# Darkkey/erlamsa

Measured on AMD Instinct MI355X. Metric: mutated_MB_per_s, higher is better.
Workload: dtype u8 (byte edits) + f64 (AS183 draws)

## Files before the change

### erlamsa_amd/csrc/eh_fuse.h

```cpp
#pragma once
#include "eh_field.h"

namespace eh {

struct FNode { uint32_t fo, fc, to, tc; };

EH_DEV uint32_t wave_sort64(uint32_t key) {
  const uint32_t l = (uint32_t)EH_LANE;
#pragma unroll
  for (uint32_t k2 = 2; k2 <= 64; k2 <<= 1) {
#pragma unroll
    for (uint32_t j = k2 >> 1; j > 0; j >>= 1) {
      uint32_t other = (uint32_t)__shfl_xor((int)key, (int)j);
      bool up = (l & k2) == 0 || k2 == 64, lower = (l & j) == 0;
      bool take_min = lower == up;
      uint32_t mn = key < other ? key : other, mx = key < other ? other : key;
      key = take_min ? mn : mx;
    }
  }
  return key;
}
EH_DEV uint32_t lanes_le(uint32_t v, uint32_t cnt, uint32_t x) {
  uint32_t lo = 0;
#pragma unroll
  for (uint32_t s = 32; s > 0; s >>= 1) { uint32_t t = (uint32_t)__shfl((int)v, (int)((lo + s - 1) & 63)); if (lo + s <= cnt && t <= x) lo += s; }
  { uint32_t t = (uint32_t)__shfl((int)v, (int)(lo & 63)); if (lo < cnt && t <= x) lo++; }
  return lo;
}
EH_DEV uint32_t lanes_lt(uint32_t v, uint32_t cnt, uint32_t x) { uint32_t r = lanes_le(v, cnt, x ? x - 1 : 0u); return x == 0 ? 0u : r; }

EH_DEV uint64_t wave_sum64(uint64_t v) {
#pragma unroll
  for (int d = 32; d > 0; d >>= 1) v += ((uint64_t)(uint32_t)__shfl_xor((int)(uint32_t)(v >> 32), d) << 32) | (uint32_t)__shfl_xor((int)(uint32_t)v, d);
  return uni64(v);
}
}
#include "eh_fuse_lds.h"
namespace eh {
#define FUSE_UNROLL 4
struct FuseGen { EH_G FNode* nd; wptr F; wptr T; };

EH_DEV uint32_t fuse_round(cbptr A, uint32_t la, cbptr B, uint32_t lb, const FuseGen& g, uint32_t nn, const FuseGen& o, uint32_t par, bool sym, uint64_t* entries) {
  const int l = EH_LANE;
  const bool asc = par == 0;
  uint64_t le = 0;
  uint32_t cn = 0, cf = 0, ct = 0;
  uint32_t k0 = 0;
  while (k0 < nn) {
    uint32_t k = k0 + (uint32_t)l;
    FNode nd = {0, 0, 0, 0};
    if (k < nn) nd = g.nd[k];
    if (sym) { nd.to = nd.fo; nd.tc = nd.fc; }
    bool valid = k < nn;
    bool big = valid && (nd.fc > 64 || nd.tc > 64);
    bool one = valid && nd.fc == 1 && nd.tc == 1;
    unsigned long long vm = __ballot(valid), bm = __ballot(big), om = __ballot(one);
    uint32_t nvalid = (uint32_t)__popcll(vm);
    uint32_t nones = ~om == 0ull ? 64u : (uint32_t)__builtin_ctzll(~om);
    if (nones > nvalid) nones = nvalid;
    if (nones >= 16 || (nones > 0 && nones == nvalid)) {
      bool in = (uint32_t)l < nones;
      uint32_t p = in ? nd.fo : la, q = in ? nd.to : lb;
      bool special = in && p == la - 1;
      bool same;
      if (sym) same = in && p < la;
      else { uint32_t ba = (in && p < la) ? A[p] : 256u, bb = (in && q < lb) ? B[q] : 257u; same = ba == bb; }
      bool child = special || same;
      bool tkeep = child && !special && q != lb - 1;
      unsigned long long cm = __ballot(child);
      uint32_t ci = (uint32_t)__popcll(cm & ((1ull << l) - 1));
      if (child) {
        FNode c2; c2.fo = special ? la : p + 1; c2.fc = 1; c2.to = special ? lb : q + 1; c2.tc = (special || tkeep) ? 1u : 0u;
        o.nd[cn + ci] = c2;
        le += 1u + c2.tc;
      }
      cn += (uint32_t)__popcll(cm);
      k0 += nones;
      continue;
    }
    if (bm & 1ull) {
      FNode b0; b0.fo = uni(nd.fo); b0.fc = uni(nd.fc); b0.to = uni(nd.to); b0.tc = uni(nd.tc);
      uint32_t* hf = g_fuse_lds; uint32_t* ht = sym ? g_fuse_lds : g_fuse_lds + 256;
      uint32_t* hc = g_fuse_lds + 512; uint32_t* hk = g_fuse_lds + 768;
      for (uint32_t i = l; i < 512; i += 64) g_fuse_lds[i] = 0;
      lanes_sync();
      uint32_t fdb = 0xFFFFFFFFu, fdbefore = 0, tdb = 0xFFFFFFFFu, tdbefore = 0;
      for (int side = 0; side < (sym ? 1 : 2); side++) {
        cbptr S = side ? B : A; uint32_t slen = side ? lb : la;
        uint32_t cnt = side ? b0.tc : b0.fc;
        cwptr P = side ? g.T + b0.to : g.F + b0.fo;
        uint32_t single = side ? b0.to : b0.fo;
        uint32_t* h = side ? ht : hf;
        for (uint32_t base = 0; base < cnt; base += 64 * FUSE_UNROLL) {
          uint32_t pp[FUSE_UNROLL], bt[FUSE_UNROLL]; bool v[FUSE_UNROLL];
#pragma unroll
          for (int u = 0; u < FUSE_UNROLL; u++) {
            uint32_t i = base + 64u * (uint32_t)u + (uint32_t)l; bool in = i < cnt;
            pp[u] = in ? (cnt == 1 ? single : P[i]) : slen; v[u] = in && pp[u] < slen;
          }
#pragma unroll
          for (int u = 0; u < FUSE_UNROLL; u++) { bt[u] = v[u] ? (uint32_t)S[pp[u]] : 0u; if (!asc) bt[u] = 255u - bt[u]; }
#pragma unroll
          for (int u = 0; u < FUSE_UNROLL; u++) {
            unsigned long long lastm = __ballot(v[u] && pp[u] == slen - 1);
            if (lastm) {
              int j = (int)__builtin_ctzll(lastm);
              uint32_t bj = (uint32_t)__builtin_amdgcn_readlane((int)bt[u], j);
              lanes_sync();
              uint32_t before = h[bj] + (uint32_t)__popcll(__ballot(v[u] && bt[u] == bj) & ((1ull << j) - 1));
              if (side) { tdb = bj; tdbefore = before; } else { fdb = bj; fdbefore = before; }
              lanes_sync();
            }
            if (v[u]) atomicAdd(&h[bt[u]], 1u);
          }
        }
      }
      if (sym) { tdb = fdb; tdbefore = fdbefore; }
      lanes_sync();
      uint32_t rf[4], rt[4], ef[4], et[4]; bool ch[4], sp[4];
      uint32_t lc = 0, lf = 0, lt2 = 0;
      bool anyfd = false, anytd = false;
#pragma unroll
      for (int j = 0; j < 4; j++) {
        uint32_t bt = 4u * (uint32_t)l + (uint32_t)j;
        rf[j] = hf[bt]; rt[j] = ht[bt];
        bool fdrop = bt == fdb && (asc ? fdbefore == 0 : fdbefore + 1 == rf[j]);
        bool tdrop = bt == tdb && (asc ? tdbefore == 0 : tdbefore + 1 == rt[j]);
        anyfd |= fdrop; anytd |= tdrop;
        ef[j] = rf[j] - (fdrop ? 1u : 0u); et[j] = rt[j] - (tdrop ? 1u : 0u);
        sp[j] = rf[j] > 0 && ef[j] == 0;
        ch[j] = rf[j] > 0 && (sp[j] || rt[j] > 0);
        if (sp[j]) { ef[j] = 1; et[j] = 1; }
        if (!ch[j]) { ef[j] = 0; et[j] = 0; }
        le += ef[j] + et[j];
        lc += ch[j] ? 1u : 0u; lf += ef[j] > 1 ? ef[j] : 0u; lt2 += et[j] > 1 ? et[j] : 0u;
      }
      const bool fdropped = __ballot(anyfd) != 0, tdropped = __ballot(anytd) != 0;
      uint32_t ic = wave_incl_scan(lc), iff = wave_incl_scan(lf), it = wave_incl_scan(lt2);
      uint32_t oc = cn + ic - lc, of = cf + iff - lf, ot = sym ? of : ct + it - lt2;
      lanes_sync();
#pragma unroll
      for (int j = 0; j < 4; j++) {
        uint32_t bt = 4u * (uint32_t)l + (uint32_t)j;
        bool scat = ch[j] && !sp[j];
        hf[bt] = scat ? of : 0xFFFFFFFFu; if (!sym) ht[bt] = scat ? ot : 0xFFFFFFFFu;
        hc[bt] = scat ? oc : 0xFFFFFFFFu; hk[bt] = (ef[j] == 1 ? 1u : 0u) | (et[j] == 1 ? 2u : 0u);
        if (ch[j]) {
          FNode c2; c2.fo = sp[j] ? la : of; c2.fc = ef[j]; c2.to = sp[j] ? lb : ot; c2.tc = et[j];
          o.nd[oc] = c2;
          oc++; if (ef[j] > 1) of += ef[j]; if (sym) ot = of; else if (et[j] > 1) ot += et[j];
        }
      }
      cn += (uint32_t)__builtin_amdgcn_readlane((int)ic, 63); cf += (uint32_t)__builtin_amdgcn_readlane((int)iff, 63); ct += (uint32_t)__builtin_amdgcn_readlane((int)it, 63);
      wave_sync();
      for (int side = 0; side < (sym ? 1 : 2); side++) {
        cbptr S = side ? B : A; uint32_t slen = side ? lb : la;
        uint32_t cnt = side ? b0.tc : b0.fc;
        cwptr P = side ? g.T + b0.to : g.F + b0.fo;
        uint32_t single = side ? b0.to : b0.fo;
        uint32_t* h = side ? ht : hf; wptr O = side ? o.T : o.F;
        const bool dropped = side ? tdropped : fdropped;
        for (uint32_t base = 0; base < cnt; base += 64 * FUSE_UNROLL) {
          uint32_t ppu[FUSE_UNROLL], btu[FUSE_UNROLL]; bool vu[FUSE_UNROLL];
#pragma unroll
          for (int u = 0; u < FUSE_UNROLL; u++) {
            uint32_t i = base + 64u * (uint32_t)u + (uint32_t)l; bool in = i < cnt;
            ppu[u] = in ? (cnt == 1 ? single : P[i]) : slen; vu[u] = in && ppu[u] < slen;
          }
#pragma unroll
          for (int u = 0; u < FUSE_UNROLL; u++) { btu[u] = vu[u] ? (uint32_t)S[ppu[u]] : 0u; if (!asc) btu[u] = 255u - btu[u]; }
#pragma unroll
          for (int u = 0; u < FUSE_UNROLL; u++) {
            const uint32_t pp = ppu[u], bt = btu[u]; const bool v = vu[u];
            if (base + 64u * (uint32_t)u >= cnt) break;
            bool isdrop = dropped && v && pp == slen - 1;
            bool vv = v && !isdrop;
            unsigned long long eq = __ballot(vv);
#pragma unroll
            for (int bit = 0; bit < 8; bit++) { unsigned long long m = __ballot(vv && ((bt >> bit) & 1u)); eq &= ((bt >> bit) & 1u) ? m : ~m; }
            uint32_t rank = (uint32_t)__popcll(eq & ((1ull << l) - 1)), cntg = (uint32_t)__popcll(eq);
            uint32_t off = vv ? h[bt] : 0xFFFFFFFFu, cidx = vv ? hc[bt] : 0xFFFFFFFFu, kf = vv ? hk[bt] : 0u;
            lanes_sync();
            if (vv && cidx != 0xFFFFFFFFu) {
              bool isone = (kf >> side) & 1u;
              if (isone) { if (side) o.nd[cidx].to = pp + 1; else { o.nd[cidx].fo = pp + 1; if (sym) o.nd[cidx].to = pp + 1; } }
              else { O[off + rank] = pp + 1; if (rank == 0) h[bt] = off + cntg; }
            }
            lanes_sync();
          }
        }
      }
      k0 += 1;
      continue;
    }
    uint32_t cumf = wave_incl_scan(valid && !big ? nd.fc : 0u), cumt = wave_incl_scan(valid && !big ? nd.tc : 0u);
    uint32_t firstbig = bm ? (uint32_t)__builtin_ctzll(bm) : 64u;
    unsigned long long fitm = __ballot(valid && (uint32_t)l < firstbig && cumf <= 64 && cumt <= 64);
    uint32_t nfit = ~fitm == 0ull ? 64u : (uint32_t)__builtin_ctzll(~fitm);
    uint32_t totf = (uint32_t)__builtin_amdgcn_readlane((int)cumf, (int)(nfit - 1)), tott = (uint32_t)__builtin_amdgcn_readlane((int)cumt, (int)(nfit - 1));
    uint32_t key[2], pos[2], tot[2] = {totf, tott};
#pragma unroll
    for (int side = 0; side < 2; side++) {
      if (side == 1 && sym) { key[1] = key[0]; pos[1] = pos[0]; break; }
      cbptr S = side ? B : A; uint32_t slen = side ? lb : la;
      uint32_t cum = side ? cumt : cumf, cntn = side ? nd.tc : nd.fc, offn = side ? nd.to : nd.fo;
      bool in = (uint32_t)l < tot[side];
      uint32_t nj = lanes_le(cum, nfit, (uint32_t)l);
      uint32_t ex = (uint32_t)__shfl((int)(cum - cntn), (int)(nj & 63)), ob = (uint32_t)__shfl((int)offn, (int)(nj & 63)), cj = (uint32_t)__shfl((int)cntn, (int)(nj & 63));
      uint32_t pp = slen;
      if (in) pp = cj == 1 ? ob : (side ? g.T : g.F)[ob + ((uint32_t)l - ex)];
      bool v = in && pp < slen;
      uint32_t bt = v ? (uint32_t)S[pp] : 0u; if (!asc) bt = 255u - bt;
      uint32_t kk = in ? (((nj << 9) | (v ? bt : 511u)) << 6) | (uint32_t)l : 0xFFFFFFFFu;
      uint32_t nxt = (uint32_t)__shfl_down((int)kk, 1);
      uint32_t sk = __ballot(l < 63 && kk > nxt) == 0 ? kk : wave_sort64(kk);
      key[side] = sk; pos[side] = (uint32_t)__shfl((int)pp, (int)(sk & 63u));
    }
    uint32_t gk[2], lead[2], len[2], drops[2]; bool alive[2], isdrop[2];
#pragma unroll
    for (int side = 0; side < 2; side++) {
      if (side == 1 && sym) { gk[1] = gk[0]; lead[1] = lead[0]; len[1] = len[0]; drops[1] = drops[0]; alive[1] = alive[0]; isdrop[1] = isdrop[0]; break; }
      uint32_t slen = side ? lb : la;
      gk[side] = key[side] >> 6;
      alive[side] = (uint32_t)l < tot[side] && (gk[side] & 511u) != 511u;
      uint32_t prevk = (uint32_t)__shfl_up((int)gk[side], 1), nextk = (uint32_t)__shfl_down((int)gk[side], 1);
      bool leader = alive[side] && (l == 0 || prevk != gk[side]);
      bool last = alive[side] && (l == 63 || (uint32_t)l + 1 >= tot[side] || nextk != gk[side]);
      unsigned long long lm = __ballot(leader);
      uint32_t ll = alive[side] ? 63u - (uint32_t)__builtin_clzll(lm & ((2ull << l) - 1)) : 0u;
      unsigned long long after = lm & ~((2ull << ll) - 1);
      unsigned long long am = __ballot(alive[side]);
      uint32_t endl = after ? (uint32_t)__builtin_ctzll(after) : 64u;
      unsigned long long dead_after = ~am & ~((2ull << ll) - 1);
      uint32_t endd = dead_after ? (uint32_t)__builtin_ctzll(dead_after) : 64u;
      uint32_t e = endl < endd ? endl : endd;
      lead[side] = ll; len[side] = alive[side] ? e - ll : 0u;
      isdrop[side] = alive[side] && pos[side] == slen - 1 && (asc ? leader : last);
      unsigned long long dm = __ballot(isdrop[side]);
      unsigned long long runm = (e >= 64 ? ~0ull : ((1ull << e) - 1)) & ~((1ull << ll) - 1);
      drops[side] = alive[side] ? (uint32_t)__popcll(dm & runm) : 0u;
    }
    uint32_t tl = sym ? lead[0] : lanes_lt(gk[1], tott, gk[0]);
    uint32_t tk_at = (uint32_t)__shfl((int)gk[1], (int)(tl & 63)), tlen_at = (uint32_t)__shfl((int)len[1], (int)(tl & 63)), tdr_at = (uint32_t)__shfl((int)drops[1], (int)(tl & 63));
    bool tldrop = __shfl((int)(isdrop[1] ? 1 : 0), (int)(tl & 63)) != 0;
    bool texists = alive[0] && tl < tott && tk_at == gk[0];
    bool fleader = alive[0] && lead[0] == (uint32_t)l;
    uint32_t fcnt = len[0] - drops[0];
    bool special = fleader && fcnt == 0;
    bool child = fleader && (special || texists);
    uint32_t nf = child ? (special ? 1u : fcnt) : 0u, nt = child ? (special ? 1u : (tlen_at - tdr_at)) : 0u;
    uint32_t af = nf > 1 ? nf : 0u, at = nt > 1 ? nt : 0u;
    uint32_t ic = wave_incl_scan(child ? 1u : 0u), iff = wave_incl_scan(af), it = wave_incl_scan(at);
    uint32_t oc = cn + ic - (child ? 1u : 0u), of = cf + iff - af, ot = sym ? of : ct + it - at;
    uint32_t fsurv = (uint32_t)__shfl((int)pos[0], (int)(((uint32_t)l + (isdrop[0] ? 1u : 0u)) & 63));
    uint32_t tsurv = (uint32_t)__shfl((int)pos[1], (int)((tl + (tldrop ? 1u : 0u)) & 63));
    if (child) {
      FNode c2;
      c2.fc = nf; c2.tc = nt;
      c2.fo = special ? la : (nf == 1 ? fsurv + 1 : of);
      c2.to = special ? lb : (nt == 1 ? tsurv + 1 : (nt == 0 ? 0u : ot));
      o.nd[oc] = c2;
      le += nf + nt;
    }
    {
      bool lmulti = __shfl((int)(child && !special && nf > 1 ? 1 : 0), (int)lead[0]) != 0;
      uint32_t lof = (uint32_t)__shfl((int)of, (int)lead[0]);
      bool ldrop = __shfl((int)(isdrop[0] ? 1 : 0), (int)lead[0]) != 0;
      if (alive[0] && lmulti && !isdrop[0]) o.F[lof + ((uint32_t)l - lead[0]) - (ldrop ? 1u : 0u)] = pos[0] + 1;
    }
    if (!sym) {
      uint32_t sl = lanes_lt(gk[0], totf, gk[1]);
      uint32_t sk_at = (uint32_t)__shfl((int)gk[0], (int)(sl & 63));
      bool has = alive[1] && sl < totf && sk_at == gk[1];
      bool smulti = __shfl((int)(child && !special && nt > 1 ? 1 : 0), (int)(sl & 63)) != 0;
      uint32_t sot = (uint32_t)__shfl((int)ot, (int)(sl & 63));
      bool ldrop = __shfl((int)(isdrop[1] ? 1 : 0), (int)lead[1]) != 0;
      if (has && smulti && !isdrop[1]) o.T[sot + ((uint32_t)l - lead[1]) - (ldrop ? 1u : 0u)] = pos[1] + 1;
    }
    cn += (uint32_t)__builtin_amdgcn_readlane((int)ic, 63); cf += (uint32_t)__builtin_amdgcn_readlane((int)iff, 63); ct += (uint32_t)__builtin_amdgcn_readlane((int)it, 63);
    k0 += nfit;
  }
  *entries = wave_sum64(le);
  wave_sync();
  return cn;
}

__device__ bool fuse_jump_stream(Ctx& c, cbptr A, uint32_t la, cbptr B, uint32_t lb, bool sym, uint32_t* from, uint32_t* tpos, uint32_t* rounds);
}
#include "eh_fuse_red.h"
namespace eh {

#ifdef EH_FUSE_INLINE
EH_DEV bool fuse_lists(Ctx& c, cbptr A, uint32_t la, cbptr B, uint32_t lb, bptr* out, uint32_t* outlen) {
#else
__device__ __noinline__ bool fuse_lists(Ctx&, cbptr A, uint32_t la, cbptr B, uint32_t lb, bptr* out, uint32_t* outlen) {
  EH_CTX;
#endif
  const int l = EH_LANE;
  if (la == 0) { *out = (bptr)B; *outlen = lb; return true; }
  if (lb == 0) { *out = (bptr)A; *outlen = la; return true; }
  uint64_t mark = c.ws_used;
  const bool sym = A == B && la == lb;
  EH_PT0;
  uint32_t from = la, tpos = lb;
  uint32_t prof_rounds = 0;
  c.fp_on = 0;
  if ((sym ? (uint64_t)la : (uint64_t)la + lb) > FL_NMAX && !c.work_budget && !(c.p->flags & EH_FLAG_FUSE_NO_REDUCE)) {
    const uint32_t rd = fr_peek_rounds(c.rng);
    if (rd < 64) {
      const uint32_t R = rd + 2u;
      uint32_t la2 = la, lb2 = lb;
      cbptr A2 = fr_reduce(c, A, &la2, R);
      if (!A2) return false;
      cbptr B2 = A2;
      if (sym) lb2 = la2; else { B2 = fr_reduce(c, B, &lb2, R); if (!B2) return false; }
      if ((uint64_t)la2 + lb2 <= ((uint64_t)la + lb) / 4u * 3u) {
        EH_PT(c, 97);
        c.fp_on = 1;
        bool ok;
        if ((sym ? (uint64_t)la2 : (uint64_t)la2 + lb2) <= FL_NMAX && !(c.p->flags & EH_FLAG_FUSE_NO_LDS)) ok = fuse_jump_lds(c, A2, la2, B2, lb2, sym, &from, &tpos, &prof_rounds);
        else ok = fuse_jump_stream(c, A2, la2, B2, lb2, sym, &from, &tpos, &prof_rounds);
        c.fp_on = 0;
        if (!ok) return false;
        EH_PT(c, 54);
        const uint32_t g = c.fp_g, par = g & 1u;
        from = la; tpos = lb;
        if (g == 0) { from = rng_rand(c.rng, la); tpos = rng_rand(c.rng, lb); }
        else if (c.fp_special) { (void)rng_rand(c.rng, 1); (void)rng_rand(c.rng, 1); }
        else {
          cbptr key = A2 + c.fp_keypos;
          const uint32_t limA = la > g ? la - g : 0u, limB = lb > g ? lb - g : 0u;
          const uint32_t fc0 = fr_occ(A, la, limA, key, g, FR_NONE, nullptr), fc = fc0 + c.fp_bA;
          uint32_t pos = 0;
          if (fc > 0) { uint32_t j = rng_rand(c.rng, fc); j = par ? fc - 1u - j : j; if (j < fc0) { (void)fr_occ(A, la, limA, key, g, j, &pos); from = uni(pos) + g; } }
          const uint32_t tc0 = sym ? fc0 : fr_occ(B, lb, limB, key, g, FR_NONE, nullptr), tc = tc0 + c.fp_bB;
          if (tc > 0) { uint32_t j = rng_rand(c.rng, tc); j = par ? tc - 1u - j : j; if (j < tc0) { (void)fr_occ(B, lb, limB, key, g, j, &pos); tpos = uni(pos) + g; } }
        }
        EH_PT(c, 55);
        goto jump;
      }
    }
    EH_PT(c, 98);
    c.ws_used = mark;
  }
  if ((sym ? (uint64_t)la : (uint64_t)la + lb) <= FL_NMAX && !(c.p->flags & EH_FLAG_FUSE_NO_LDS)) {
    if (!fuse_jump_lds(c, A, la, B, lb, sym, &from, &tpos, &prof_rounds)) { if (c.status == CASE_BUDGET) c.ws_used = mark; return false; }
  } else if ((uint64_t)la + lb >= c.p->fuse_stream_min) {
    if (!fuse_jump_stream(c, A, la, B, lb, sym, &from, &tpos, &prof_rounds)) { if (c.status == CASE_BUDGET) c.ws_used = mark; return false; }
  } else {
    FuseGen g[2];
    for (int k = 0; k < 2; k++) {
      g[k].nd = (EH_G FNode*)ws_alloc(c, ((uint64_t)la + 4) * sizeof(FNode));
      g[k].F = (wptr)ws_alloc(c, ((uint64_t)la + 4) * 4);
      g[k].T = sym ? g[k].F : (wptr)ws_alloc(c, ((uint64_t)lb + 4) * 4);
      if (!g[k].nd || !g[k].F || !g[k].T) return false;
    }
    if (la > 1) for (uint32_t i = l; i < la; i += 64) g[0].F[i] = i;
    if (lb > 1 && !sym) for (uint32_t i = l; i < lb; i += 64) g[0].T[i] = i;
    if (l == 0) { FNode n0; n0.fo = 0; n0.fc = la; n0.to = 0; n0.tc = lb; g[0].nd[0] = n0; }
    uint32_t nn = 1, par = 0;
    int64_t fuel = 100000;
    uint64_t gen_entries = (uint64_t)la + lb;
    wave_sync();
    while (true) {
      if (fuel < 0) break;
      if (rng_rand(c.rng, 8) == 0) break;
      if (c.work_budget) {
        c.work += 16ull * gen_entries;
        if (c.work > c.work_budget) { c.status = CASE_BUDGET; c.ws_used = mark; return false; }
      }
      uint32_t nchild = fuse_round(A, la, B, lb, g[par], nn, g[par ^ 1], par, sym, &gen_entries);
      if (nchild == 0) break;
      par ^= 1; nn = nchild;
      fuel -= (int64_t)nchild;
      prof_rounds++;
    }
    uint32_t ni = rng_rand(c.rng, nn);
    FNode nd = g[par].nd[par ? nn - 1 - ni : ni];
    uint32_t fo = uni(nd.fo), fc = uni(nd.fc), to = sym ? fo : uni(nd.to), tc = sym ? fc : uni(nd.tc);
    if (fc > 0) { uint32_t j = rng_rand(c.rng, fc); from = fc == 1 ? fo : uni(g[par].F[fo + (par ? fc - 1 - j : j)]); }
    if (tc > 0) { uint32_t j = rng_rand(c.rng, tc); tpos = tc == 1 ? to : uni(g[par].T[to + (par ? tc - 1 - j : j)]); }
  }
jump:
#ifdef EH_PROF
  {
    uint32_t tot = la + lb, b = 0; while ((256u << b) < tot && b < 13) b++;
    EH_PT(c, 112 + b);
    if (EH_LANE == 0) { atomicAdd(&c.p->prof[2 * 126], (unsigned long long)prof_rounds); atomicAdd(&c.p->prof[2 * 126 + 1], 1ull); }
  }
#endif
  c.ws_used = mark;
  uint32_t nl = from + (lb - tpos);
  bptr dst = ws_alloc(c, nl);
  if (!dst) return false;
  wave_copy(dst, A, from);
  wave_copy(dst + from, B + tpos, lb - tpos);
  wave_sync();
  *out = dst; *outlen = nl;
  return true;
}

struct FoState { uint64_t ptr; uint32_t len; uint32_t has; };

__device__ __noinline__ int muta_fuse(Ctx&, int fn, EH_G FoState* fo) {
  EH_CTX;
  Blk hb = blk_load(c.bl, c.cur);
  cbptr H = (cbptr)hb.ptr; uint32_t L = hb.len;
  c.r_kind = R_SAME;
  bptr r; uint32_t rl;
  if (fn == M_FT) {
    if (!fuse_lists(c, H, L, H, L, &r, &rl)) return 0;
    int d = rng_delta(c.rng);
    c.r_kind = R_NEW; c.r_ptr = r; c.r_len = rl;
    return d;
  }
  uint32_t h1 = L / 2;
  if (fn == M_FN) {
    Blk nb = hb; bool have_next = c.cur + 1 < c.nb;
    if (have_next) nb = blk_load(c.bl, c.cur + 1);
    bptr abl; uint32_t abll;
    if (!fuse_lists(c, H, h1, (cbptr)nb.ptr, nb.len, &abl, &abll)) return 0;
    if (!fuse_lists(c, abl, abll, H + h1, L - h1, &r, &rl)) return 0;
    int d = rng_delta(c.rng);
    c.r_kind = R_NEW; c.r_ptr = r; c.r_len = rl; c.r_flush = 1; c.r_drop_next = have_next ? 1 : 0;
    return d;
  }
  uint32_t has = uni(fo->has);
  uint64_t optr = has ? uni64(fo->ptr) : hb.ptr; uint32_t olen = has ? uni(fo->len) : L;
  uint32_t o1 = olen / 2;
  bptr a; uint32_t al; bptr b; uint32_t bl;
  if (!fuse_lists(c, H, h1, (cbptr)optr, o1, &a, &al)) return 0;
  if (!fuse_lists(c, (cbptr)optr + o1, olen - o1, H + h1, L - h1, &b, &bl)) return 0;
  uint32_t swap = rng_rand(c.rng, 3);
  int d = rng_delta(c.rng);
  if (EH_LANE == 0) { if (!has || swap == 0) { fo->ptr = hb.ptr; fo->len = L; } fo->has = 1; }
  wave_sync();
  c.r_kind = R_NEW; c.r_ptr = a; c.r_len = al; c.r_flush = 1;
  c.r2_ptr = b; c.r2_len = bl; c.r2 = 1;
  return d;
}

}
```

### erlamsa_amd/engine.py

```python
import ctypes as C
import os

import numpy as np

_HERE = os.path.dirname(os.path.abspath(__file__))
LIB_PATH = os.environ.get("ERLAMSA_HIP_LIB") or os.path.join(_HERE, "liberlamsa_hip.so")

EH_ABI_VERSION = 8
EH_FLAG_ORDERED_OUTPUT = 1
EH_FLAG_META_TRACE = 2
EH_FLAG_FUSE_NO_LDS = 4
EH_FLAG_FUSE_NO_REDUCE = 8
EH_FLAG_SGML_NO_REPLAY = 16
EH_FLAG_SGML_NO_LANES = 32
EH_FLAG_NO_COOP = 64

UNIQUE_PIECE_BYTES = 65536

CASE_OK, CASE_CRASHED, CASE_OVERFLOW, CASE_UNSUPPORTED, CASE_ARENA_FULL, CASE_BUDGET = 0, 1, 2, 3, 4, 5

ABI_SYMBOLS = [
    "eh_create", "eh_destroy", "eh_configure", "eh_corpus_upload", "eh_corpus_attach", "eh_fuzz_batch",
    "eh_fuzz_calls", "eh_reserve", "eh_sync", "eh_result_device", "eh_result_download", "eh_result_fetch", "eh_result_totals", "eh_result_summary", "eh_result_occupancy", "eh_result_diag", "eh_result_cycles", "eh_result_peak", "eh_result_meta", "eh_result_write_files", "eh_result_prof", "eh_selftest_movers", "eh_selftest_zlib",
    "eh_last_kernel_ms", "eh_pool_stats", "eh_coop_stats", "eh_kernel_name", "eh_abi_version", "eh_mutator_count", "eh_mutator_name",
    "eh_mutator_default_pri", "eh_mutator_on_gpu", "eh_pattern_count", "eh_pattern_name",
    "eh_pattern_default_pri", "eh_pattern_on_gpu", "eh_strerror", "eh_last_error",
    "eh_coalesce_limits", "eh_submit", "eh_flush", "eh_poll", "eh_cancel",
    "eh_corpus_device", "eh_stream", "eh_host_alloc", "eh_host_free", "eh_selftest_sort_by_priority", "eh_last_error_copy",
    "eh_comm_unique_id", "eh_comm_init", "eh_comm_init_local", "eh_comm_destroy", "eh_corpus_broadcast", "eh_corpus_allgather",
    "eh_corpus_broadcast_local", "eh_device_count", "eh_meta_atom_count", "eh_meta_atom_name", "eh_batch_done",
    "eh_result_digests", "eh_result_unique", "eh_result_download_select", "eh_selftest_unique",
    "eh_profile_add", "eh_profile_count", "eh_fuzz_calls_profiled", "eh_submit_profiled",
    "eh_seen_reserve", "eh_seen_count", "eh_seen_add_keys", "eh_seen_add_corpus", "eh_seen_export", "eh_result_seen", "eh_selftest_seen",
]

SEEN_FRESH, SEEN_IN_BATCH, SEEN_BEFORE, SEEN_NOT_OK = 0, 1, 2, 3

MAX_PROFILES = 1024


class EhOptions(C.Structure):
    _fields_ = [("abi_version", C.c_uint32), ("mutations", C.c_char_p), ("patterns", C.c_char_p),
                ("generators", C.c_char_p), ("blockscale", C.c_double), ("ssrf_host", C.c_char_p),
                ("ssrf_port", C.c_int32), ("max_case_bytes", C.c_uint64), ("out_capacity", C.c_uint64),
                ("max_case_work", C.c_uint64), ("max_slots", C.c_uint32), ("flags", C.c_uint32), ("big_case_bytes", C.c_uint64),
                ("pool_bytes", C.c_uint64), ("download_chunk_bytes", C.c_uint64), ("fuse_stream_min", C.c_uint64),
                ("sequence_muta", C.c_uint32), ("reserved0", C.c_uint32)]


class EngineError(RuntimeError):
    def __init__(self, code, msg):
        super().__init__("erlamsa_hip error %d: %s" % (code, msg))
        self.code = code


_lib = None


def load_library():
    global _lib
    if _lib is not None:
        return _lib
    import sys
    if "torch" in sys.modules:
        import torch
        if torch.cuda.is_available():
            torch.cuda.init()
    if not os.path.exists(LIB_PATH):
        raise ImportError("%s not built: run `python -c 'import __graft_entry__ as g; g.build()'`" % LIB_PATH)
    lib = C.CDLL(LIB_PATH)
    vp, u64p, i64p, i32p = C.c_void_p, C.POINTER(C.c_uint64), C.POINTER(C.c_int64), C.POINTER(C.c_int32)
    lib.eh_create.argtypes = [C.c_int, C.POINTER(vp)]
    lib.eh_destroy.argtypes = [vp]
    lib.eh_destroy.restype = None
    lib.eh_configure.argtypes = [vp, C.POINTER(EhOptions)]
    lib.eh_corpus_upload.argtypes = [vp, vp, vp, C.c_uint64]
    lib.eh_corpus_attach.argtypes = [vp, vp, vp, C.c_uint64, C.c_uint64]
    lib.eh_fuzz_batch.argtypes = [vp, i64p, C.c_uint64, C.c_uint64, C.c_uint64, vp]
    lib.eh_fuzz_calls.argtypes = [vp, vp, C.c_uint64, C.c_uint64, vp]
    lib.eh_sync.argtypes = [vp]
    lib.eh_batch_done.argtypes = [vp, C.POINTER(C.c_int)]
    lib.eh_reserve.argtypes = [vp, C.c_uint64]
    lib.eh_result_device.argtypes = [vp, C.POINTER(vp), C.POINTER(vp), C.POINTER(vp), C.POINTER(vp), u64p]
    lib.eh_result_download.argtypes = [vp, vp, C.c_uint64, vp, vp]
    lib.eh_result_totals.argtypes = [vp, u64p, u64p, u64p]
    lib.eh_result_fetch.argtypes = [vp, C.c_uint64, vp, C.c_uint64, u64p]
    lib.eh_result_diag.argtypes = [vp, vp, vp]
    lib.eh_result_cycles.argtypes = [vp, vp]
    lib.eh_result_peak.argtypes = [vp, vp]
    lib.eh_result_write_files.argtypes = [vp, C.c_char_p, C.c_uint64, C.c_uint32, u64p, u64p, u64p]
    lib.eh_result_meta.argtypes = [vp, C.c_uint64, vp, C.c_uint64, u64p]
    lib.eh_result_prof.argtypes = [vp, vp]
    lib.eh_selftest_movers.argtypes = [vp, vp, C.c_uint64, vp, C.c_uint32, vp]
    lib.eh_selftest_zlib.argtypes = [vp, C.c_int, vp, C.c_uint64, vp, C.c_uint64, vp, vp]
    lib.eh_result_digests.argtypes = [vp, vp]
    lib.eh_result_unique.argtypes = [vp, vp, u64p, u64p]
    lib.eh_result_download_select.argtypes = [vp, vp, C.c_uint64, vp, C.c_uint64, vp]
    lib.eh_selftest_unique.argtypes = [vp, vp, vp, vp, C.c_uint64, vp, vp]
    lib.eh_seen_reserve.argtypes = [vp, C.c_uint64]
    lib.eh_seen_count.argtypes = [vp, vp]
    lib.eh_seen_add_keys.argtypes = [vp, vp, C.c_uint64, u64p]
    lib.eh_seen_add_corpus.argtypes = [vp, u64p]
    lib.eh_seen_export.argtypes = [vp, vp, C.c_uint64, u64p]
    lib.eh_result_seen.argtypes = [vp, C.c_uint32, vp, u64p, u64p]
    lib.eh_selftest_seen.argtypes = [vp, vp, vp, vp, C.c_uint64, C.c_uint32, vp]
    lib.eh_last_kernel_ms.argtypes = [vp, C.POINTER(C.c_float)]
    lib.eh_pool_stats.argtypes = [vp, vp]
    lib.eh_result_summary.argtypes = [vp, vp]
    lib.eh_result_occupancy.argtypes = [vp, vp]
    lib.eh_coop_stats.argtypes = [vp, vp]
    lib.eh_coalesce_limits.argtypes = [vp, C.c_uint64, C.c_uint64]
    lib.eh_submit.argtypes = [vp, vp, C.c_uint64, i64p, u64p]
    lib.eh_flush.argtypes = [vp]
    lib.eh_profile_add.argtypes = [vp, C.c_char_p, C.c_char_p, C.c_double, C.POINTER(C.c_uint32)]
    lib.eh_profile_count.argtypes = [vp, C.POINTER(C.c_uint32)]
    lib.eh_fuzz_calls_profiled.argtypes = [vp, vp, vp, C.c_uint64, C.c_uint64, vp]
    lib.eh_submit_profiled.argtypes = [vp, vp, C.c_uint64, i64p, C.c_uint32, u64p]
    lib.eh_meta_atom_name.restype = C.c_char_p
    lib.eh_meta_atom_name.argtypes = [C.c_int]
    lib.eh_comm_unique_id.argtypes = [vp]
    lib.eh_comm_init.argtypes = [vp, vp, C.c_int, C.c_int]
    lib.eh_comm_init_local.argtypes = [vp, C.c_int]
    lib.eh_comm_destroy.argtypes = [vp]
    lib.eh_corpus_broadcast.argtypes = [vp, C.c_int, vp, vp, C.c_uint64]
    lib.eh_corpus_allgather.argtypes = [vp, vp, vp, C.c_uint64]
    lib.eh_corpus_broadcast_local.argtypes = [vp, C.c_int, C.c_int]
    lib.eh_cancel.argtypes = [vp, C.c_uint64]
    lib.eh_poll.argtypes = [vp, C.c_uint64, vp, C.c_uint64, u64p, C.POINTER(C.c_int32)]
    lib.eh_corpus_device.argtypes = [vp, C.POINTER(vp), C.POINTER(vp), u64p, u64p]
    lib.eh_stream.argtypes = [vp, C.POINTER(vp)]
    lib.eh_host_alloc.argtypes = [C.POINTER(vp), C.c_uint64]
    lib.eh_host_free.argtypes = [vp]
    lib.eh_host_free.restype = None
    lib.eh_selftest_sort_by_priority.argtypes = [vp, C.c_uint32, vp]
    lib.eh_kernel_name.restype = C.c_char_p
    lib.eh_abi_version.restype = C.c_uint32
    for f in ("eh_mutator_name", "eh_pattern_name", "eh_strerror"):
        getattr(lib, f).restype = C.c_char_p
        getattr(lib, f).argtypes = [C.c_int]
    lib.eh_last_error.restype = C.c_char_p
    lib.eh_last_error.argtypes = [vp]
    _lib = lib
    return lib


def mutator_table():
    lib = load_library()
    return [(lib.eh_mutator_name(i).decode(), lib.eh_mutator_default_pri(i), bool(lib.eh_mutator_on_gpu(i)))
            for i in range(lib.eh_mutator_count())]


def pattern_table():
    lib = load_library()
    return [(lib.eh_pattern_name(i).decode(), lib.eh_pattern_default_pri(i), bool(lib.eh_pattern_on_gpu(i)))
            for i in range(lib.eh_pattern_count())]


def sort_by_priority(pris):
    p = np.ascontiguousarray(pris, dtype=np.uint32)
    perm = np.zeros(max(len(p), 1), dtype=np.uint32)
    rc = load_library().eh_selftest_sort_by_priority(p.ctypes.data, len(p), perm.ctypes.data)
    if rc != 0:
        raise EngineError(rc, "eh_selftest_sort_by_priority")
    return [int(x) for x in perm[:len(p)]]


def gpu_mutators():
    return [n for n, _, g in mutator_table() if g]


def gpu_patterns():
    return [n for n, _, g in pattern_table() if g]


class Engine:

    def __init__(self, device=0):
        self.lib = load_library()
        h = C.c_void_p()
        rc = self.lib.eh_create(device, C.byref(h))
        if rc != 0:
            raise EngineError(rc, self.lib.eh_strerror(rc).decode())
        self.h = h
        self._keep = []
        self.n_corpus = 0
        self.last_n = 0

    def close(self):
        if self.h:
            self.lib.eh_destroy(self.h)
            self.h = None

    def __del__(self):
        try:
            self.close()
        except Exception:
            pass

    def _chk(self, rc):
        if rc != 0:
            raise EngineError(rc, self.lib.eh_last_error(self.h).decode() or self.lib.eh_strerror(rc).decode())

    def configure(self, mutations=None, patterns=None, generators=None, blockscale=1.0, ssrf_host=None, ssrf_port=0,
                  max_case_bytes=0, out_capacity=0, max_slots=0, flags=0, max_case_work=0, big_case_bytes=0,
                  pool_bytes=0, download_chunk_bytes=0, fuse_stream_min=0, sequence_muta=False):
        o = EhOptions()
        o.sequence_muta = 1 if sequence_muta else 0
        o.abi_version = EH_ABI_VERSION
        o.mutations = mutations.encode() if mutations is not None else None
        o.patterns = patterns.encode() if patterns is not None else None
        o.generators = generators.encode() if generators is not None else None
        o.blockscale = blockscale
        o.ssrf_host = ssrf_host.encode() if ssrf_host else None
        o.ssrf_port = ssrf_port
        o.max_case_bytes = max_case_bytes
        o.big_case_bytes = big_case_bytes
        o.pool_bytes, o.download_chunk_bytes, o.fuse_stream_min = pool_bytes, download_chunk_bytes, fuse_stream_min
        o.out_capacity = out_capacity
        o.max_slots = max_slots
        o.max_case_work = max_case_work
        o.flags = flags
        self._chk(self.lib.eh_configure(self.h, C.byref(o)))

    def upload_corpus(self, data, off):
        data = np.ascontiguousarray(data, dtype=np.uint8)
        off = np.ascontiguousarray(off, dtype=np.uint64)
        n = len(off) - 1
        self._chk(self.lib.eh_corpus_upload(self.h, data.ctypes.data, off.ctypes.data, n))
        self.n_corpus = n

    def attach_corpus(self, d_data_ptr, d_off_ptr, n, nbytes):
        self._chk(self.lib.eh_corpus_attach(self.h, C.c_void_p(d_data_ptr), C.c_void_p(d_off_ptr), n, nbytes))
        self.n_corpus = n

    @staticmethod
    def comm_unique_id():
        lib = load_library()
        buf = (C.c_uint8 * 128)()
        rc = lib.eh_comm_unique_id(buf)
        if rc != 0:
            raise EngineError(rc, lib.eh_strerror(rc).decode() + " (RCCL could not be loaded: EH_RCCL_LIB)")
        return bytes(buf)

    def comm_init(self, unique_id, rank, nranks):
        buf = (C.c_uint8 * 128).from_buffer_copy(unique_id)
        self._chk(self.lib.eh_comm_init(self.h, buf, rank, nranks))

    def comm_destroy(self):
        self._chk(self.lib.eh_comm_destroy(self.h))

    def corpus_broadcast(self, root, data=None, off=None):
        if data is not None:
            data = np.ascontiguousarray(data, dtype=np.uint8)
            off = np.ascontiguousarray(off, dtype=np.uint64)
            self._chk(self.lib.eh_corpus_broadcast(self.h, root, data.ctypes.data, off.ctypes.data, len(off) - 1))
        else:
            self._chk(self.lib.eh_corpus_broadcast(self.h, root, None, None, 0))
        self.n_corpus = self.corpus_device()[2]

    def corpus_allgather(self, data, off):
        data = np.ascontiguousarray(data, dtype=np.uint8)
        off = np.ascontiguousarray(off, dtype=np.uint64)
        self._chk(self.lib.eh_corpus_allgather(self.h, data.ctypes.data, off.ctypes.data, len(off) - 1))
        self.n_corpus = self.corpus_device()[2]

    @staticmethod
    def comm_init_local(engines):
        arr = (C.c_void_p * len(engines))(*[e.h for e in engines])
        rc = engines[0].lib.eh_comm_init_local(arr, len(engines))
        engines[0]._chk(rc)

    @staticmethod
    def corpus_broadcast_local(engines, root=0):
        arr = (C.c_void_p * len(engines))(*[e.h for e in engines])
        rc = engines[0].lib.eh_corpus_broadcast_local(arr, len(engines), root)
        engines[root]._chk(rc)
        for e in engines:
            e.n_corpus = engines[root].n_corpus

    def corpus_device(self):
        d, o, n, nb = C.c_void_p(), C.c_void_p(), C.c_uint64(), C.c_uint64()
        self._chk(self.lib.eh_corpus_device(self.h, C.byref(d), C.byref(o), C.byref(n), C.byref(nb)))
        return d.value, o.value, n.value, nb.value

    def share_corpus(self, other):
        d, o, n, nb = other.corpus_device()
        self.attach_corpus(d, o, n, nb)
        self._keep.append(other)

    def own_stream(self):
        s = C.c_void_p()
        self._chk(self.lib.eh_stream(self.h, C.byref(s)))
        return s.value or 0

    def fuzz_batch(self, seed=(1, 2, 3), first_case=1, corpus_first=0, n=None, stream=0):
        if n is None:
            n = self.n_corpus - corpus_first
        s = (C.c_int64 * 3)(*seed)
        self._chk(self.lib.eh_fuzz_batch(self.h, s, first_case, corpus_first, n, C.c_void_p(stream)))
        self.last_n = n

    def fuzz_calls(self, seeds, profiles=None, corpus_first=0, stream=0):
        seeds = np.ascontiguousarray(seeds, dtype=np.int64).reshape(-1)
        n = seeds.size // 3
        if profiles is None:
            self._chk(self.lib.eh_fuzz_calls(self.h, seeds.ctypes.data, corpus_first, n, C.c_void_p(stream)))
        else:
            ids = np.ascontiguousarray(profiles, dtype=np.uint32).reshape(-1)
            if ids.size != n:
                raise ValueError("fuzz_calls: %d profile ids for %d seeds" % (ids.size, n))
            self._chk(self.lib.eh_fuzz_calls_profiled(self.h, seeds.ctypes.data, ids.ctypes.data, corpus_first, n, C.c_void_p(stream)))
        self.last_n = n

    def profile_add(self, mutations=None, patterns=None, blockscale=1.0):
        pid = C.c_uint32()
        self._chk(self.lib.eh_profile_add(self.h, mutations.encode() if mutations is not None else None,
                                          patterns.encode() if patterns is not None else None, float(blockscale), C.byref(pid)))
        return pid.value
# ... 300 lines not shown
```

### include/erlamsa_hip.h

```cpp
#ifndef ERLAMSA_HIP_H
#define ERLAMSA_HIP_H
#include <stdint.h>
#ifdef __cplusplus
extern "C" {
#endif

#define EH_ABI_VERSION 8

typedef struct eh_ctx eh_ctx;

enum eh_error {
  EH_OK = 0,
  EH_E_INVALID = -1,
  EH_E_NODEVICE = -2,
  EH_E_HIP = -3,
  EH_E_NOMEM = -4,
  EH_E_STATE = -5,
  EH_E_UNSUPPORTED = -6,
  EH_E_AGAIN = -7
};

enum eh_case_status {
  EH_CASE_OK = 0,
  EH_CASE_CRASHED = 1,
  EH_CASE_OVERFLOW = 2,
  EH_CASE_UNSUPPORTED = 3,
  EH_CASE_ARENA_FULL = 4,
  EH_CASE_BUDGET = 5
};

typedef struct eh_options {
  uint32_t abi_version;
  const char* mutations;
  const char* patterns;
  const char* generators;
  double blockscale;
  const char* ssrf_host;
  int32_t ssrf_port;
  uint64_t max_case_bytes;
  uint64_t out_capacity;
  uint64_t max_case_work;
  uint32_t max_slots;
  uint32_t flags;
  uint64_t big_case_bytes;
  uint64_t pool_bytes;
  uint64_t download_chunk_bytes;
  uint64_t fuse_stream_min;
  uint32_t sequence_muta;
  uint32_t reserved0;
} eh_options;

#define EH_FLAG_NO_COOP 64u
#define EH_FLAG_TREE_NO_LANES 128u
#define EH_FLAG_ORDERED_OUTPUT 1u
#define EH_FLAG_META_TRACE 2u
#define EH_FLAG_SGML_NO_LANES 32u
#define EH_FLAG_SGML_NO_REPLAY 16u
#define EH_FLAG_FUSE_NO_REDUCE 8u
#define EH_FLAG_FUSE_NO_LDS 4u

int eh_create(int device, eh_ctx** out);
void eh_destroy(eh_ctx* ctx);
int eh_configure(eh_ctx* ctx, const eh_options* opts);

int eh_corpus_upload(eh_ctx* ctx, const uint8_t* data, const uint64_t* off, uint64_t n);
int eh_corpus_attach(eh_ctx* ctx, const void* d_data, const void* d_off, uint64_t n, uint64_t nbytes);

int eh_device_count(void);
int eh_comm_unique_id(uint8_t id[128]);
int eh_comm_init(eh_ctx* ctx, const uint8_t id[128], int rank, int nranks);
int eh_comm_init_local(eh_ctx** ctxs, int nctx);
int eh_comm_destroy(eh_ctx* ctx);
int eh_corpus_broadcast(eh_ctx* ctx, int root, const uint8_t* data, const uint64_t* off, uint64_t n);
int eh_corpus_allgather(eh_ctx* ctx, const uint8_t* data, const uint64_t* off, uint64_t n_local);
int eh_corpus_broadcast_local(eh_ctx** ctxs, int nctx, int root);

int eh_corpus_device(eh_ctx* ctx, const void** d_data, const void** d_off, uint64_t* n, uint64_t* nbytes);

int eh_stream(eh_ctx* ctx, void** stream);

int eh_host_alloc(void** p, uint64_t bytes);
void eh_host_free(void* p);

int eh_reserve(eh_ctx* ctx, uint64_t max_cases);

int eh_fuzz_batch(eh_ctx* ctx, const int64_t seed[3], uint64_t first_case, uint64_t corpus_first, uint64_t n,
                  void* stream);
int eh_fuzz_calls(eh_ctx* ctx, const int64_t* seeds, uint64_t corpus_first, uint64_t n, void* stream);
int eh_sync(eh_ctx* ctx);
int eh_batch_done(eh_ctx* ctx, int* done);

int eh_coalesce_limits(eh_ctx* ctx, uint64_t flush_cases, uint64_t flush_bytes);
int eh_submit(eh_ctx* ctx, const uint8_t* data, uint64_t len, const int64_t seed[3], uint64_t* ticket);
int eh_flush(eh_ctx* ctx);
int eh_poll(eh_ctx* ctx, uint64_t ticket, uint8_t* out, uint64_t cap, uint64_t* out_len, int32_t* status);
int eh_cancel(eh_ctx* ctx, uint64_t ticket);

#define EH_MAX_PROFILES 1024
int eh_profile_add(eh_ctx* ctx, const char* mutations, const char* patterns, double blockscale, uint32_t* id);
int eh_profile_count(eh_ctx* ctx, uint32_t* n);
int eh_fuzz_calls_profiled(eh_ctx* ctx, const int64_t* seeds, const uint32_t* profile, uint64_t corpus_first, uint64_t n, void* stream);
int eh_submit_profiled(eh_ctx* ctx, const uint8_t* data, uint64_t len, const int64_t seed[3], uint32_t profile, uint64_t* ticket);

int eh_result_device(eh_ctx* ctx, const uint8_t** d_data, const uint64_t** d_off, const uint64_t** d_len,
                     const int32_t** d_status, uint64_t* total_bytes);
int eh_result_download(eh_ctx* ctx, uint8_t* data, uint64_t cap, uint64_t* off, int32_t* status);
int eh_result_fetch(eh_ctx* ctx, uint64_t i, uint8_t* buf, uint64_t cap, uint64_t* out_len);
int eh_result_totals(eh_ctx* ctx, uint64_t* in_bytes, uint64_t* out_bytes, uint64_t* n_cases);
int eh_result_summary(eh_ctx* ctx, uint64_t* out);
int eh_result_occupancy(eh_ctx* ctx, uint64_t* out);
int eh_result_diag(eh_ctx* ctx, uint64_t* draws, int32_t* last_mutator);

int eh_result_cycles(eh_ctx* ctx, uint64_t* cycles);

int eh_result_write_files(eh_ctx* ctx, const char* name_template, uint64_t first_number, uint32_t threads,
                          uint64_t* files_written, uint64_t* bytes_written, uint64_t* not_written);

int eh_meta_atom_count(void);
const char* eh_meta_atom_name(int id);
int eh_result_meta(eh_ctx* ctx, uint64_t i, uint8_t* buf, uint64_t cap, uint64_t* n_events);

#define EH_UNIQUE_PIECE_BYTES 65536
int eh_result_digests(eh_ctx* ctx, uint64_t* digest);
int eh_result_unique(eh_ctx* ctx, uint64_t* first_of, uint64_t* n_unique, uint64_t* unique_bytes);
int eh_result_download_select(eh_ctx* ctx, const uint64_t* idx, uint64_t m, uint8_t* data, uint64_t cap, uint64_t* off);
int eh_selftest_unique(eh_ctx* ctx, const uint8_t* data, const uint64_t* off, const int32_t* status, uint64_t n,
                       uint64_t* digest, uint64_t* first_of);

int eh_seen_reserve(eh_ctx* ctx, uint64_t capacity);
int eh_seen_count(eh_ctx* ctx, uint64_t out[4]);
int eh_seen_add_keys(eh_ctx* ctx, const uint64_t* keys, uint64_t m, uint64_t* added);
int eh_seen_add_corpus(eh_ctx* ctx, uint64_t* added);
int eh_seen_export(eh_ctx* ctx, uint64_t* keys, uint64_t cap_keys, uint64_t* n);
int eh_result_seen(eh_ctx* ctx, uint32_t commit, uint8_t* cls, uint64_t* n_fresh, uint64_t* fresh_bytes);
int eh_selftest_seen(eh_ctx* ctx, const uint8_t* data, const uint64_t* off, const int32_t* status, uint64_t n, uint32_t commit,
                     uint8_t* cls);

int eh_result_peak(eh_ctx* ctx, uint64_t* peak);

int eh_result_prof(eh_ctx* ctx, uint64_t* prof);

int eh_selftest_movers(eh_ctx* ctx, uint8_t* buf, uint64_t buf_len, const uint32_t* jobs, uint32_t njobs, uint32_t* eq_out);
int eh_selftest_zlib(eh_ctx* ctx, int op, const uint8_t* in, uint64_t n, uint8_t* out, uint64_t cap, uint64_t* out_len, int32_t* ok);

int eh_selftest_sort_by_priority(const uint32_t* pri, uint32_t n, uint32_t* perm);

int eh_pool_stats(eh_ctx* ctx, uint64_t* out);
int eh_coop_stats(eh_ctx* ctx, uint64_t* out);

int eh_last_kernel_ms(eh_ctx* ctx, float* ms);
const char* eh_kernel_name(void);

uint32_t eh_abi_version(void);
int eh_mutator_count(void);
const char* eh_mutator_name(int id);
int eh_mutator_default_pri(int id);
int eh_mutator_on_gpu(int id);
int eh_pattern_count(void);
const char* eh_pattern_name(int id);
int eh_pattern_default_pri(int id);
int eh_pattern_on_gpu(int id);
const char* eh_strerror(int code);
const char* eh_last_error(eh_ctx* ctx);
uint64_t eh_last_error_copy(eh_ctx* ctx, char* buf, uint64_t cap);

#ifdef __cplusplus
}
#endif
#endif
```

Measured before the change: 78560.

## Add direct hash-table fast path for symmetric fuse jump selection

```diff
diff --git a/erlamsa_amd/csrc/eh_fuse.h b/erlamsa_amd/csrc/eh_fuse.h
--- a/erlamsa_amd/csrc/eh_fuse.h
+++ b/erlamsa_amd/csrc/eh_fuse.h
@@ -288,6 +288,7 @@
 __device__ bool fuse_jump_stream(Ctx& c, cbptr A, uint32_t la, cbptr B, uint32_t lb, bool sym, uint32_t* from, uint32_t* tpos, uint32_t* rounds);
 }
 #include "eh_fuse_red.h"
+#include "eh_fuse_direct.h"
 namespace eh {
 
 #ifdef EH_FUSE_INLINE
@@ -318,7 +319,7 @@
         EH_PT(c, 97);
         c.fp_on = 1;
         bool ok;
-        if ((sym ? (uint64_t)la2 : (uint64_t)la2 + lb2) <= FL_NMAX && !(c.p->flags & EH_FLAG_FUSE_NO_LDS)) ok = fuse_jump_lds(c, A2, la2, B2, lb2, sym, &from, &tpos, &prof_rounds);
+        if ((sym ? (uint64_t)la2 : (uint64_t)la2 + lb2) <= FL_NMAX && !(c.p->flags & EH_FLAG_FUSE_NO_LDS)) ok = fuse_jump_direct(c, A2, la2, B2, lb2, sym, &from, &tpos, &prof_rounds) || fuse_jump_lds(c, A2, la2, B2, lb2, sym, &from, &tpos, &prof_rounds);
         else ok = fuse_jump_stream(c, A2, la2, B2, lb2, sym, &from, &tpos, &prof_rounds);
         c.fp_on = 0;
         if (!ok) return false;
@@ -344,7 +345,7 @@
     c.ws_used = mark;
   }
   if ((sym ? (uint64_t)la : (uint64_t)la + lb) <= FL_NMAX && !(c.p->flags & EH_FLAG_FUSE_NO_LDS)) {
-    if (!fuse_jump_lds(c, A, la, B, lb, sym, &from, &tpos, &prof_rounds)) { if (c.status == CASE_BUDGET) c.ws_used = mark; return false; }
+    if (!fuse_jump_direct(c, A, la, B, lb, sym, &from, &tpos, &prof_rounds) && !fuse_jump_lds(c, A, la, B, lb, sym, &from, &tpos, &prof_rounds)) { if (c.status == CASE_BUDGET) c.ws_used = mark; return false; }
   } else if ((uint64_t)la + lb >= c.p->fuse_stream_min) {
     if (!fuse_jump_stream(c, A, la, B, lb, sym, &from, &tpos, &prof_rounds)) { if (c.status == CASE_BUDGET) c.ws_used = mark; return false; }
   } else {
diff --git a/erlamsa_amd/csrc/eh_fuse_direct.h b/erlamsa_amd/csrc/eh_fuse_direct.h
--- /dev/null
+++ b/erlamsa_amd/csrc/eh_fuse_direct.h
@@ -0,0 +1,225 @@
+#pragma once
+#define EH_FUSE_DIRECT_MAX_LA 4528
+
+namespace eh {
+
+constexpr uint32_t FD_H_OFF = EH_FUSE_LDS_WORDS - 256u;
+constexpr uint32_t FD_EMPTY = 0xFFFFu, FD_NONE = 0xFFFFFFFFu;
+constexpr uint32_t FD_DB_MAX = (EH_FUSE_DIRECT_MAX_LA + 31u) & ~15u;
+static_assert((FD_H_OFF * 4u - FD_DB_MAX) / 2u >= 3u * EH_FUSE_DIRECT_MAX_LA / 2u, "eh_fuse_direct.h: 1.5 table slots per position");
+static_assert(EH_FUSE_DIRECT_MAX_LA < FD_EMPTY && EH_FUSE_DIRECT_MAX_LA <= FL_NMAX, "eh_fuse_direct.h: positions are 16 bits");
+
+#ifdef HIPEMU
+extern "C" { inline unsigned long long eh_emu_fuse_direct[5] = {0, 0, 0, 0, 0}; }
+#define FD_COUNT(i) do { if (EH_LANE == 0) eh_emu_fuse_direct[i] += 1; } while (0)
+#else
+#define FD_COUNT(i) do { } while (0)
+#endif
+
+struct FdLay { const uint8_t* D; uint16_t* Tb; uint32_t* H; uint32_t T; };
+
+EH_DEV uint32_t fd_bytep(uint32_t b, uint32_t d) { return (d & 1u) ? 255u - b : b; }
+EH_DEV uint64_t fd_ld8(const uint8_t* D, uint32_t p) {
+  const uint32_t* W = reinterpret_cast<const uint32_t*>(D) + (p >> 2);
+  const uint32_t w0 = W[0], w1 = W[1], w2 = W[2], sh = 8u * (p & 3u);
+  const uint64_t lo = ((uint64_t)w1 << 32) | w0;
+  return sh ? (lo >> sh) | ((uint64_t)w2 << (64u - sh)) : lo;
+}
+EH_DEV uint64_t fd_chunk(const uint8_t* D, uint32_t p, uint32_t j, uint32_t R) {
+  const uint32_t rem = R - 8u * j;
+  const uint64_t v = fd_ld8(D, p + 8u * j);
+  return rem >= 8u ? v : v & ((1ull << (8u * rem)) - 1ull);
+}
+EH_DEV uint32_t fd_hash(const uint8_t* D, uint32_t p, uint32_t R) {
+  uint32_t h = 2166136261u;
+  for (uint32_t j = 0; 8u * j < R; j++) {
+    const uint64_t v = fd_chunk(D, p, j, R);
+    h = (h ^ (uint32_t)v) * 0x9E3779B1u;
+    h = (h ^ (h >> 15) ^ (uint32_t)(v >> 32)) * 0x85EBCA77u;
+  }
+  h ^= h >> 13; h *= 0xC2B2AE3Du; h ^= h >> 16;
+  return h;
+}
+EH_DEV bool fd_same(const uint8_t* D, uint32_t p, uint32_t q, uint32_t R) {
+  uint64_t diff = 0;
+  for (uint32_t j = 0; 8u * j < R; j++) diff |= fd_chunk(D, p, j, R) ^ fd_chunk(D, q, j, R);
+  return diff == 0;
+}
+
+EH_DEV bool fd_insert(const FdLay& y, uint32_t R, uint32_t lo, uint32_t hi, uint32_t* nrep) {
+  const uint32_t l = (uint32_t)EH_LANE;
+  uint32_t p = lo + l, reps = 0, probes = 0;
+  bool pend = p < hi, fail = false;
+  uint32_t slot = pend ? (uint32_t)(((uint64_t)fd_hash(y.D, p, R) * y.T) >> 32) : 0u;
+  while (__ballot(pend) != 0) {
+    if (__ballot(fail) != 0) return false;
+    if (pend && (uint32_t)y.Tb[slot] == FD_EMPTY) y.Tb[slot] = (uint16_t)p;
+    wave_sync();
+    if (pend) {
+      const uint32_t occ = (uint32_t)y.Tb[slot];
+      bool done = true;
+      if (occ == p) { reps++; atomicAdd(&y.H[(uint32_t)y.D[p]], 1u); }
+      else if (!fd_same(y.D, p, occ, R)) { done = false; slot = slot + 1u == y.T ? 0u : slot + 1u; if (++probes > y.T) { fail = true; pend = false; } }
+      if (done) {
+        p += 64u; probes = 0; pend = p < hi;
+        if (pend) slot = (uint32_t)(((uint64_t)fd_hash(y.D, p, R) * y.T) >> 32);
+      }
+    }
+  }
+  if (__ballot(fail) != 0) return false;
+  *nrep += wave_sum(reps);
+  return true;
+}
+EH_DEV bool fd_lookup(const FdLay& y, uint32_t R, uint32_t q) {
+  uint32_t slot = (uint32_t)(((uint64_t)fd_hash(y.D, q, R) * y.T) >> 32);
+  for (uint32_t tries = 0; tries <= y.T; tries++) {
+    const uint32_t occ = (uint32_t)y.Tb[slot];
+    if (occ == FD_EMPTY) return false;
+    if (fd_same(y.D, q, occ, R)) return true;
+    slot = slot + 1u == y.T ? 0u : slot + 1u;
+  }
+  return false;
+}
+EH_DEV uint32_t fd_bin_of(const uint32_t* H, uint32_t k, uint32_t* before, uint32_t* cnt) {
+  const uint32_t l = (uint32_t)EH_LANE;
+  const uint32_t h0 = H[4u * l], h1 = H[4u * l + 1u], h2 = H[4u * l + 2u], h3 = H[4u * l + 3u];
+  const uint32_t s = h0 + h1 + h2 + h3, inc = wave_incl_scan(s), ex = inc - s;
+  const bool mine = k >= ex && k < inc;
+  uint32_t b = 4u * l, bef = ex, n = h0;
+  if (k >= bef + n) { bef += n; b++; n = h1; }
+  if (b == 4u * l + 1u && k >= bef + n) { bef += n; b++; n = h2; }
+  if (b == 4u * l + 2u && k >= bef + n) { bef += n; b++; n = h3; }
+  const unsigned long long who = __ballot(mine);
+  const int src = who ? (int)__builtin_ctzll(who) : 0;
+  *before = (uint32_t)__builtin_amdgcn_readlane((int)bef, src);
+  *cnt = (uint32_t)__builtin_amdgcn_readlane((int)n, src);
+  return (uint32_t)__builtin_amdgcn_readlane((int)b, src);
+}
+EH_DEV uint32_t fd_keep_bin(const FdLay& y, uint32_t n, uint32_t d, uint32_t b) {
+  const uint32_t l = (uint32_t)EH_LANE;
+  uint32_t w = 0;
+  for (uint32_t base = 0; base < n; base += 256) {
+    uint32_t e[4]; bool keep[4]; unsigned long long km[4];
+#pragma unroll
+    for (int u = 0; u < 4; u++) { const uint32_t i = base + 64u * (uint32_t)u + l; e[u] = i < n ? (uint32_t)y.Tb[i] : FD_EMPTY; }
+#pragma unroll
+    for (int u = 0; u < 4; u++) keep[u] = e[u] != FD_EMPTY && fd_bytep((uint32_t)y.D[(e[u] != FD_EMPTY ? e[u] : 0u) + d], d) == b;
+#pragma unroll
+    for (int u = 0; u < 4; u++) km[u] = __ballot(keep[u]);
+    lanes_sync();
+#pragma unroll
+    for (int u = 0; u < 4; u++) {
+      if (keep[u]) y.Tb[w + (uint32_t)__popcll(km[u] & ((1ull << l) - 1ull))] = (uint16_t)e[u];
+      w += (uint32_t)__popcll(km[u]);
+    }
+    lanes_sync();
+  }
+  wave_sync();
+  return w;
+}
+EH_DEV uint32_t fd_occ(const uint8_t* D, uint32_t q, uint32_t R, uint32_t lim, uint32_t w1, uint32_t w2, uint32_t* p1, uint32_t* p2) {
+  const uint32_t l = (uint32_t)EH_LANE;
+  const bool stop = w1 != FD_NONE || w2 != FD_NONE;
+  bool need1 = w1 != FD_NONE, need2 = w2 != FD_NONE;
+  uint32_t seen = 0;
+  for (uint32_t base = 0; base < lim; base += 256) {
+    bool hit[4];
+#pragma unroll
+    for (int u = 0; u < 4; u++) { const uint32_t p = base + 64u * (uint32_t)u + l; hit[u] = p < lim && fd_same(D, p < lim ? p : 0u, q, R); }
+#pragma unroll
+    for (int u = 0; u < 4; u++) {
+      const uint32_t b0 = base + 64u * (uint32_t)u;
+      const unsigned long long m = __ballot(hit[u]);
+      const uint32_t rank = seen + (uint32_t)__popcll(m & ((1ull << l) - 1ull));
+      const unsigned long long m1 = __ballot(hit[u] && need1 && rank == w1), m2 = __ballot(hit[u] && need2 && rank == w2);
+      if (m1) { *p1 = b0 + (uint32_t)__builtin_ctzll(m1); need1 = false; }
+      if (m2) { *p2 = b0 + (uint32_t)__builtin_ctzll(m2); need2 = false; }
+      seen += (uint32_t)__popcll(m);
+    }
+    if (stop && !need1 && !need2) break;
+  }
+  return seen;
+}
+
+__device__ __noinline__ bool fuse_jump_direct(Ctx&, cbptr A, uint32_t la, cbptr B, uint32_t lb, bool sym, uint32_t* from, uint32_t* tpos, uint32_t* rounds) {
+  EH_CTX;
+  (void)B; (void)lb;
+  const uint32_t l = (uint32_t)EH_LANE;
+  if (!sym || c.work_budget || (c.p->flags & (EH_FLAG_FUSE_NO_LDS | EH_FLAG_FUSE_NO_DIRECT))) return false;
+  const uint32_t R = fr_peek_rounds(c.rng);
+  if (R < 1u || R >= 64u) return false;
+  EH_PT0;
+  if ((uint64_t)R * la > 100000u) { FD_COUNT(1); EH_PT(c, 47); return false; }
+  if (la > EH_FUSE_DIRECT_MAX_LA) { FD_COUNT(2); EH_PT(c, 47); return false; }
+  if (la < R + 2u) { FD_COUNT(3); EH_PT(c, 47); return false; }
+  const uint32_t db = (la + 31u) & ~15u;
+  const uint32_t avail = (FD_H_OFF * 4u - db) / 2u, wish = (2u * la + 64u) & ~7u;
+  FdLay y;
+  uint8_t* Dw = reinterpret_cast<uint8_t*>(g_fuse_lds);
+  y.D = Dw; y.Tb = reinterpret_cast<uint16_t*>(Dw + db); y.H = g_fuse_lds + FD_H_OFF; y.T = wish < avail ? wish : avail;
+  lanes_sync();
+  {
+    uint32_t k = 16u * l;
+    for (; k + 16u <= la; k += 1024u) { const uint4 v = ldg16(A + k); uint32_t* w = g_fuse_lds + (k >> 2); w[0] = v.x; w[1] = v.y; w[2] = v.z; w[3] = v.w; }
+    for (uint32_t t = (la & ~15u) + l; t < db; t += 64) Dw[t] = t < la ? A[t] : (uint8_t)0;
+    uint32_t* tw = g_fuse_lds + (db >> 2);
+    for (uint32_t t = l; t < (y.T + 1u) / 2u; t += 64) tw[t] = 0xFFFFFFFFu;
+    for (uint32_t t = l; t < 256u; t += 64) y.H[t] = 0;
+  }
+  wave_sync();
+  const uint32_t star = la - R;
+  uint32_t nn = 0;
+  if (!fd_insert(y, R, 0, star, &nn)) { FD_COUNT(4); EH_PT(c, 47); return false; }
+  wave_sync();
+  const bool star_alone = !uni(fd_lookup(y, R, star) ? 1u : 0u);
+  if (star_alone && !fd_insert(y, R, star, star + 1u, &nn)) { FD_COUNT(4); EH_PT(c, 47); return false; }
+  wave_sync();
+  FD_COUNT(0);
+  rng_skip(c.rng, R + 1u);
+  *rounds += R;
+  const uint32_t par = R & 1u;
+  const uint32_t ni = rng_rand(c.rng, nn);
+  uint32_t k = par ? nn - 1u - ni : ni;
+  uint32_t n = y.T;
+  for (uint32_t d = 0; d < R; d++) {
+    if (d > 0) {
+      if (n <= 1u) break;
+      for (uint32_t t = l; t < 256u; t += 64) y.H[t] = 0;
+      wave_sync();
+      for (uint32_t base = 0; base < n; base += 64) if (base + l < n) atomicAdd(&y.H[fd_bytep((uint32_t)y.D[(uint32_t)y.Tb[base + l] + d], d)], 1u);
+      wave_sync();
+    }
+    uint32_t before = 0, cnt = 0;
+    const uint32_t b = fd_bin_of(y.H, k, &before, &cnt);
+    k -= before;
+    n = fd_keep_bin(y, n, d, b);
+  }
+  const uint32_t q = uni((uint32_t)y.Tb[0]);
+  const bool star_here = uni(fd_same(y.D, q, star, R) ? 1u : 0u) != 0;
+  const bool special = star_here && star_alone, star_last = star_here && !star_alone && ((R - 1u) & 1u) == 0;
+  if (c.fp_on) {
+    uint32_t e0 = star, e1 = 0;
+    if (!special) (void)fd_occ(y.D, q, R, star, 0u, FD_NONE, &e0, &e1);
+    c.fp_g = R; c.fp_keypos = uni(e0);
+    c.fp_special = special ? 1u : 0u;
+    c.fp_bA = (special || star_last) ? 1u : 0u;
+    c.fp_bB = c.fp_bA;
+    EH_PT(c, 46);
+    return true;
+  }
+  *from = la; *tpos = la;
+  if (special) { (void)rng_rand(c.rng, 1); (void)rng_rand(c.rng, 1); }
+  else {
+    uint32_t p1 = 0, p2 = 0;
+    const uint32_t fc0 = fd_occ(y.D, q, R, star, FD_NONE, FD_NONE, &p1, &p2), fc = fc0 + (star_last ? 1u : 0u);
+    const uint32_t j1 = rng_rand(c.rng, fc), j2 = rng_rand(c.rng, fc);
+    const uint32_t i1 = par ? fc - 1u - j1 : j1, i2 = par ? fc - 1u - j2 : j2;
+    p1 = p2 = star;
+    if (i1 < fc0 || i2 < fc0) (void)fd_occ(y.D, q, R, star, i1 < fc0 ? i1 : FD_NONE, i2 < fc0 ? i2 : FD_NONE, &p1, &p2);
+    *from = uni(p1) + R; *tpos = uni(p2) + R;
+  }
+  EH_PT(c, 46);
+  return true;
+}
+
+}
diff --git a/erlamsa_amd/engine.py b/erlamsa_amd/engine.py
--- a/erlamsa_amd/engine.py
+++ b/erlamsa_amd/engine.py
@@ -14,6 +14,7 @@
 EH_FLAG_SGML_NO_REPLAY = 16
 EH_FLAG_SGML_NO_LANES = 32
 EH_FLAG_NO_COOP = 64
+EH_FLAG_FUSE_NO_DIRECT = 256
 
 UNIQUE_PIECE_BYTES = 65536
 
diff --git a/include/erlamsa_hip.h b/include/erlamsa_hip.h
--- a/include/erlamsa_hip.h
+++ b/include/erlamsa_hip.h
@@ -57,6 +57,7 @@
 #define EH_FLAG_SGML_NO_LANES 32u
 #define EH_FLAG_SGML_NO_REPLAY 16u
 #define EH_FLAG_FUSE_NO_REDUCE 8u
+#define EH_FLAG_FUSE_NO_DIRECT 256u
 #define EH_FLAG_FUSE_NO_LDS 4u
 
 int eh_create(int device, eh_ctx** out);
```

Result: no change. 78240 (-0.4%).
